# krylea/stylegan3-editing

Measured on AMD Instinct MI355X. Metric: FFHQ-1024 StyleGAN3-T synthesis imgs/sec, higher is better.
Workload: dtype f32

## Files before the change

### include/sg3_ops.h

```cpp
#ifndef SG3_OPS_H
#define SG3_OPS_H

#include <stdint.h>

#ifdef __cplusplus
extern "C" {
#endif

#define SG3_ABI_VERSION 1

#if defined(__GNUC__)
#define SG3_API __attribute__((visibility("default")))
#else
#define SG3_API
#endif

enum {
    SG3_OK          =  0,
    SG3_NO_KERNEL   = -1,
    SG3_BAD_ARG     = -2,
    SG3_HIP_ERROR   = -3,
};

enum {
// ... 18 lines not shown
    int32_t        xH, xW;
    int32_t        yH, yW;
    int64_t        xStride[4];
    int64_t        yStride[4];
    int64_t        bStride;
    int32_t        up, down;
    int32_t        fuW, fuH;
    int32_t        fdW, fdH;
    int32_t        px0, py0;
    int32_t        sH;
    int32_t        sWbytes;
    int32_t        sx, sy;
    int32_t        swLimit;
    float          gain;
    float          slope;
    float          clamp;
    int32_t        flip;
    int32_t        writeSigns;
    int32_t        readSigns;
    float*         ySumPartial;
    int32_t        fdMirror;
    float*         yAbsMaxPartial;
} sg3_filtered_lrelu_params;

SG3_API int sg3_filtered_lrelu(const sg3_filtered_lrelu_params* p, void* stream);

SG3_API int sg3_filtered_lrelu_sum_slots(int N, int C, int yH, int yW, int down);

SG3_API int sg3_filtered_lrelu_finish_partials(const float* sumPartial, const float* absMaxPartial, int N, int C, int slots,
                                               float* db, float* absMax, void* stream);

SG3_API int sg3_filtered_lrelu_planes_per_wave(const sg3_filtered_lrelu_params* p);

SG3_API int sg3_filtered_lrelu_has_kernel(int up, int down, int fuW, int fuH, int fdW, int fdH);

SG3_API int sg3_filtered_lrelu_shape(int xH, int xW, int up, int down,
                             int fuW, int fuH, int fdW, int fdH,
                             int px0, int px1, int py0, int py1,
                             int* yH, int* yW,
                             int* sH, int* sWbytes, int* swLimit);

typedef struct sg3_filtered_lrelu_act_params {
    void*          x;
    uint8_t*       s;
    int32_t        dtype;
    int32_t        N, C, H, W;
    int64_t        xStride[4];
    int32_t        sH, sW;
    int32_t        sx, sy;
    float          gain, slope, clamp;
    int32_t        writeSigns;
    int32_t        readSigns;
} sg3_filtered_lrelu_act_params;

SG3_API int sg3_filtered_lrelu_act(const sg3_filtered_lrelu_act_params* p, void* stream);

typedef struct sg3_upfirdn2d_params {
    const void*    x;
    const float*   f;
    void*          y;
    int32_t        dtype;
    int32_t        N, C, xH, xW, yH, yW;
    int64_t        xStride[4];
    int64_t        yStride[4];
    int32_t        fH, fW;
    int64_t        fStride[2];
// ... 244 lines not shown
```

### stylegan3-editing_amd/csrc/sg3_filtered_lrelu.hip

```cpp
#include "sg3_common.h"
#include <cmath>
#include <cstdlib>

#ifndef SG3_PREFETCH_ROWS
#define SG3_PREFETCH_ROWS 3
#endif
#ifndef SG3_NAN_GUARD
#define SG3_NAN_GUARD 1
#endif

namespace sg3 {

typedef float v2f __attribute__((ext_vector_type(2)));
typedef float v4f __attribute__((ext_vector_type(4)));
typedef __attribute__((address_space(3))) float lds_f;
typedef __attribute__((address_space(3))) v2f lds_v2f;
typedef __attribute__((address_space(3))) v4f lds_v4f;

struct StreamParams {
    const void* x; void* y; const void* b; const float* fu; const float* fd;
    int C, xH, xW, yH, yW;
    int planes;
    long long xsN, xsC, xsH;
    long long ysN, ysC, ysH;
    long long bStride;
    int px0, py0;
    int TW;
    int ox0Base;
    int wideBlocks;
    int CH;
    int nStrips, nChunks;
    int totalBlocks;
    float gain, slope, clamp;
    int flip;
    float* ysum;
    float* ymax;
    unsigned char* s;
    int sH, sWb, sx, sy;
#ifdef SG3_STAMPS
    unsigned long long* stamps;
#endif
};
#ifdef SG3_STAMPS
static unsigned long long* g_stamps = nullptr;
#endif

__device__ __forceinline__ int to_sgpr_i(int v) { return __builtin_amdgcn_readfirstlane(v); }
__device__ __forceinline__ float to_sgpr(float v) {
    return __builtin_bit_cast(float, __builtin_amdgcn_readfirstlane(__builtin_bit_cast(int, v)));
}

__device__ __forceinline__ void wave_lds_sync() {
    __builtin_amdgcn_fence(__ATOMIC_RELEASE, "wavefront");
    __builtin_amdgcn_wave_barrier();
    __builtin_amdgcn_fence(__ATOMIC_ACQUIRE, "wavefront");
}

__device__ __forceinline__ v2f fma2(v2f a, v2f b, v2f c) { return __builtin_elementwise_fma(a, b, c); }
__device__ __forceinline__ v2f splat(float a) { return (v2f){a, a}; }

template <int HALF>
__device__ __forceinline__ v2f fma_tap(v2f a, v2f tapPair, v2f acc) {
    if (HALF == 0) return fma2(a, __builtin_shufflevector(tapPair, tapPair, 0, 0), acc);
    v2f r;
    asm("v_pk_fma_f32 %0, %1, %2, %3 op_sel:[0,1,0] op_sel_hi:[1,1,1]" : "=v"(r) : "v"(a), "s"(tapPair), "v"(acc));
    return r;
}
// ... 96 lines not shown
template <> struct bufio<_Float16> {
    static __device__ __forceinline__ float ld(__amdgpu_buffer_rsrc_t r, int byteOff) {
        return (float)__builtin_bit_cast(_Float16, __builtin_amdgcn_raw_buffer_load_b16(r, byteOff, 0, 0));
    }
    static __device__ __forceinline__ void st1(__amdgpu_buffer_rsrc_t r, int byteOff, float v) {
        __builtin_amdgcn_raw_buffer_store_b16(__builtin_bit_cast(unsigned short, (_Float16)v), r, byteOff, 0, 0);
    }
    static __device__ __forceinline__ void st2(__amdgpu_buffer_rsrc_t r, int byteOff, float a, float b) {
        const unsigned lo = __builtin_bit_cast(unsigned short, (_Float16)a), hi = __builtin_bit_cast(unsigned short, (_Float16)b);
        __builtin_amdgcn_raw_buffer_store_b32(lo | (hi << 16), r, byteOff, 0, 0);
    }
};

template <typename T, int U, int D>
struct WaveState {
    typedef StreamCfg<U, D> Cfg;
    v2f w[6][2];
    v2f xw[6][4];
    v2f acc[6][2];
    float pre[SG3_PREFETCH_ROWS][Cfg::NL];
    float bcol[Cfg::NL];
    int coff[Cfg::NL];
    v2f tuP[Cfg::FU / 2];
    v2f tdP[Cfg::FD / 2];
    unsigned sg[SG3_PREFETCH_ROWS][U];
    float osum;
    float omax;
    int soff;
    int sq;
    int inBase, outBase;
    int ooff[2];
};

template <typename T, int U, int D, int VPH, int RADIAL, int SIGNS, int G = 1>
struct Stream {
    typedef StreamCfg<U, D> Cfg;
    typedef WaveState<T, U, D> State;

    static __device__ __forceinline__ void prefetch(State& st, int slot, const StreamParams& p, const T* __restrict__ plane,
                                                    const unsigned char* __restrict__ splane, int i) {
        const bool rowOk = (unsigned)i < (unsigned)p.xH;
        const T* row = plane + (long long)i * p.xsH;
        const int rowBytes = (G > 1 ? (int)p.xsC + p.xW : p.xW) * (int)sizeof(T);
        const __amdgpu_buffer_rsrc_t rs = __builtin_amdgcn_make_buffer_rsrc((void*)row, (short)0, rowOk ? rowBytes : 0, 0x00020000);
        const float rowFlag = rowOk ? 1.f : 0.f;
#pragma unroll
        for (int q = 0; q < Cfg::NL; q++)
            st.pre[slot][q] = __builtin_fmaf(st.bcol[q], rowFlag, bufio<T>::ld(rs, st.coff[q]));
        if (SIGNS == 2) {
#pragma unroll
            for (int j = 0; j < U; j++) {
                const int sr = U * (i - 5) - (U - 1) + j + p.py0 + p.sy;
                const bool ok = (unsigned)sr < (unsigned)p.sH;
                const unsigned char* srow = splane + (ok ? (long long)sr * p.sWb : 0);
                const __amdgpu_buffer_rsrc_t ss = __builtin_amdgcn_make_buffer_rsrc((void*)srow, (short)0, ok ? p.sWb : 0, 0x00020000);
                const unsigned b0 = __builtin_amdgcn_raw_buffer_load_b8(ss, st.soff, 0, 0);
                const unsigned b1 = __builtin_amdgcn_raw_buffer_load_b8(ss, st.soff + 1, 0, 0);
                st.sg[slot][j] = b0 | (b1 << 8);
            }
        }
    }

    template <int S>
    static __device__ __forceinline__ void step(State& st, const StreamParams& p, const T* __restrict__ plane, T* __restrict__ oplane,
                                                unsigned char* __restrict__ splane, lds_f* sIn, lds_f* sOut, int i, int delta, int lane,
                                                int oy0, int oy1, int ox0, int oxN, bool pairStore, float& liveGain, float& liveGain1, bool wide) {
        constexpr bool RDOWN = RADIAL == 1 || RADIAL == 2 || RADIAL >= 5;
        constexpr bool FOLD = RADIAL >= 5;
        constexpr bool UP2D = RADIAL == 3 || RADIAL == 4;
        wave_lds_sync();
        constexpr int PS = S % SG3_PREFETCH_ROWS;
#pragma unroll
        for (int q = 0; q < Cfg::NL; q++) sIn[lane + 64 * q] = st.pre[PS][q];
        if (SIGNS == 0 && SG3_NAN_GUARD && G > 1) {
#pragma unroll
            for (int q = 0; q < Cfg::NL; q++) {
                unsigned long long m;
                asm("v_cmp_class_f32 %0, %1, %2" : "=s"(m) : "v"(st.pre[PS][q]), "s"(0x207));
                const int n0 = Cfg::PSEG - 64 * q;
                const unsigned long long first = n0 >= 64 ? ~0ull : (n0 <= 0 ? 0ull : ((1ull << (n0 & 63)) - 1ull));
                const unsigned long long mw = q < Cfg::NL - 1 ? m : 0ull;
                liveGain = (wide ? mw : (m & first)) != 0ull ? __builtin_bit_cast(float, 0x7fc00000u) : liveGain;
                liveGain1 = (wide ? mw : (m & ~first)) != 0ull ? __builtin_bit_cast(float, 0x7fc00000u) : liveGain1;
            }
        } else if (SIGNS == 0 && SG3_NAN_GUARD) {
#pragma unroll
            for (int q = 0; q < Cfg::NL - 1; q++) {
                unsigned long long m;
                asm("v_cmp_class_f32 %0, %1, %2" : "=s"(m) : "v"(st.pre[PS][q]), "s"(0x207));
                liveGain = m != 0ull ? __builtin_bit_cast(float, 0x7fc00000u) : liveGain;
            }
        }
        unsigned sgNow[U];
#pragma unroll
        for (int j = 0; j < U; j++) sgNow[j] = SIGNS == 2 ? st.sg[PS][j] : 0u;
        prefetch(st, PS, p, plane, splane, i + SG3_PREFETCH_ROWS);
        wave_lds_sync();
        if (U == 2) {
            float xs[8];
            const volatile lds_v2f* src = reinterpret_cast<const volatile lds_v2f*>(sIn + (G > 1 ? st.inBase : 2 * lane));
#pragma unroll
            for (int q = 0; q < 4; q++) { v2f t = src[q]; xs[2 * q] = t.x; xs[2 * q + 1] = t.y; if (UP2D) st.xw[S][q] = t; }
#pragma unroll
            for (int g = 0; g < 2 && !UP2D; g++) {
                v2f a = splat(xs[g]) * st.tuP[0];
#pragma unroll
                for (int t = 1; t < 6; t++) a = fma2(splat(xs[g + t]), st.tuP[t], a);
                st.w[S][g] = a;
            }
        } else {
            float xs[6];
#pragma unroll
            for (int t = 0; t < 6; t++) xs[t] = sIn[(G > 1 ? st.inBase : lane) + t];
            v2f a0 = splat(xs[0]) * st.tuP[1], a1 = splat(xs[0]) * st.tuP[0];
#pragma unroll
            for (int t = 1; t < 6; t++) {
                a0 = fma2(splat(xs[t]), st.tuP[2 * t + 1], a0);
                a1 = fma2(splat(xs[t]), st.tuP[2 * t], a1);
            }
            st.w[S][0] = a0; st.w[S][1] = a1;
        }
        const float slope = p.slope, clampv = p.clamp / p.gain, gain = p.gain;
        const float gainOut = (SIGNS == 1) ? 1.f : (UP2D ? p.gain * (float)(U * U) : ((SIGNS == 0 && SG3_NAN_GUARD) ? ((G > 1 && lane >= 32) ? liveGain1 : liveGain) : p.gain));
#pragma unroll
        for (int j = 0; j < U; j++) {
            const int kv = U - 1 - j;
            v2f u0, u1;
            TapHalf th[6];
            if (FOLD) {
                const int kp0 = (VPH + S * U + j) % D;
#pragma unroll
                for (int r = 0; r < 6; r++) radial_half_issue(th[r], p.fd, (RADIAL == 6) ? kp0 + r * D : 11 - (kp0 + r * D));
            }
            if (UP2D) {
                constexpr bool FLIPU = RADIAL == 4;
                u0 = splat(0.f); u1 = splat(0.f);
                TapRow rowA, rowB;
                radial_row_issue(rowA, p.fu, FLIPU ? kv : 11 - kv);
#pragma unroll
                for (int t = 0; t < 6; t++) {
                    const int slot = (S + 1 + t) % 6;
                    const int k = kv + 2 * t;
                    TapRow& cur = (t & 1) ? rowB : rowA;
                    TapRow& nxt = (t & 1) ? rowA : rowB;
                    radial_row_wait(cur);
                    if (t < 5) radial_row_issue(nxt, p.fu, FLIPU ? k + 2 : 11 - (k + 2));
#pragma unroll
                    for (int sx = 0; sx < 6; sx++) {
                        const v2f tq = up2d_pair<FLIPU>(cur, sx);
                        u0 = (sx & 1) ? fma_x_tap<1, FLIPU>(st.xw[slot][sx / 2], tq, u0) : fma_x_tap<0, FLIPU>(st.xw[slot][sx / 2], tq, u0);
                        u1 = ((sx + 1) & 1) ? fma_x_tap<1, FLIPU>(st.xw[slot][(sx + 1) / 2], tq, u1) : fma_x_tap<0, FLIPU>(st.xw[slot][(sx + 1) / 2], tq, u1);
                    }
                }
            }
#pragma unroll
            for (int t = 0; t < 6 && !UP2D; t++) {
// ... 8 lines not shown
                } else {
                    u0 = fma_tap<1>(st.w[slot][0], st.tuP[k / 2], u0);
                    u1 = fma_tap<1>(st.w[slot][1], st.tuP[k / 2], u1);
                }
            }
            const int uy = U * (i - 5) - (U - 1) + j + p.py0;
            float a[4] = {u0.x, u0.y, u1.x, u1.y};
            if (SIGNS == 2) {
                const unsigned bits = sgNow[j] >> (2 * st.sq);
#pragma unroll
                for (int c = 0; c < 4; c++) {
                    const unsigned code = bits >> (2 * c);
                    a[c] *= (code & 2u) ? 0.f : ((code & 1u) ? slope : 1.f);
                }
            } else if (SIGNS == 1) {
                unsigned code = 0;
#pragma unroll
                for (int c = 0; c < 4; c++) {
                    const float v = a[c] * gain;
                    const bool neg = v < 0.f;
                    const float lv = neg ? v * slope : v;
                    const bool big = __builtin_fabsf(lv) > p.clamp;
                    a[c] = big ? __builtin_copysignf(p.clamp, lv) : lv;
                    code |= (big ? 2u : (neg ? 1u : 0u)) << (2 * c);
                }
                const int sr = uy + p.sy;
                if (uy >= oy0 * D && uy <= (oy1 - 1) * D + Cfg::FD - 1 && (unsigned)sr < (unsigned)p.sH) {
                    const unsigned nxt = (unsigned)__shfl_down((int)code, 1);
                    const unsigned byte = st.sq == 0 ? code : ((code >> (2 * (4 - st.sq))) | (nxt << (2 * st.sq))) & 0xffu;
                    const int bofs = (st.sq == 0 || lane < 63) ? st.soff + (st.sq ? 1 : 0) : -1;
                    const __amdgpu_buffer_rsrc_t ss = __builtin_amdgcn_make_buffer_rsrc((void*)(splane + (long long)sr * p.sWb), (short)0, p.sWb, 0x00020000);
                    __builtin_amdgcn_raw_buffer_store_b8((unsigned char)byte, ss, bofs, 0, 0);
                }
            } else {
                const v2f s0 = u0 * splat(slope), s1 = u1 * splat(slope);
                a[0] = __builtin_fmaxf(u0.x, s0.x); a[1] = __builtin_fmaxf(u0.y, s0.y); a[2] = __builtin_fmaxf(u1.x, s1.x); a[3] = __builtin_fmaxf(u1.y, s1.y);
#pragma unroll
                for (int c = 0; c < 4; c++) a[c] = __builtin_amdgcn_fmed3f(a[c], -clampv, clampv);
            }
            const v2f r0 = {a[0], a[1]}, r1 = {a[2], a[3]};
            const int kp = (VPH + S * U + j) % D;
            if (RDOWN) {
                lds_f* dstr = sOut + (4 - delta) + (G > 1 ? st.outBase : 4 * lane);
                dstr[0] = r0.x; dstr[1] = r0.y; dstr[2] = r1.x; dstr[3] = r1.y;
                wave_lds_sync();
                const lds_v4f* srcr = reinterpret_cast<const lds_v4f*>(sOut + 4 + (G > 1 ? st.outBase : 4 * lane));
                v2f pr[8];
#pragma unroll
                for (int q = 0; q < 4; q++) { const v4f t = srcr[q]; pr[2 * q] = (v2f){t.x, t.y}; pr[2 * q + 1] = (v2f){t.z, t.w}; }
                wave_lds_sync();
                const int headR = ((VPH + S * U + j) / D) % 6;
                constexpr bool FLIPPED = RADIAL == 2 || RADIAL == 6;
                v2f fo[2][3];
#pragma unroll
                for (int q = 0; q < 3 && FOLD; q++) { fo[0][q] = add_swapped(pr[q], pr[5 - q]); fo[1][q] = add_swapped(pr[q + 1], pr[6 - q]); }
                if (FOLD) radial_half_wait(th);
#pragma unroll
                for (int r = 0; r < 6 && FOLD; r++) {
                    const int slot = (headR + 5 - r) % 6;
                    const int k = kp + r * D;
#pragma unroll
                    for (int q = 0; q < 3; q++) {
                        const v2f tq = q == 0 ? (v2f){th[r].a.x, th[r].a.y} : (q == 1 ? (v2f){th[r].a.z, th[r].a.w} : th[r].b);
                        if (k == 0 && q == 0) {
                            st.acc[slot][0] = radial_mul<true>(fo[0][0], tq);
                            st.acc[slot][1] = radial_mul<true>(fo[1][0], tq);
// ... 94 lines not shown
                        } else {
                            asm volatile("" :: "v"(f0), "v"(f1));
                        }
                        if (false) {
#else
                        if (pairStore) {
#endif
                            bufio<T>::st2(rs, G > 1 ? st.ooff[0] : 2 * lane * (int)sizeof(T), f0, f1);
                        } else {
                            bufio<T>::st1(rs, G > 1 ? st.ooff[0] : 2 * lane * (int)sizeof(T), f0);
                            bufio<T>::st1(rs, G > 1 ? st.ooff[1] : (2 * lane + 1) * (int)sizeof(T), f1);
                        }
                    } else {
                        v2f pr[12];
#pragma unroll
                        for (int q = 0; q < 6; q++) { const v4f t = src[q]; pr[2 * q] = (v2f){t.x, t.y}; pr[2 * q + 1] = (v2f){t.z, t.w}; }
                        v2f y0 = pr[0] * st.tdP[0];
#pragma unroll
                        for (int q = 1; q < Cfg::FD / 2; q++) y0 = fma2(pr[q], st.tdP[q], y0);
                        const float f0 = (y0.x + y0.y) * gainOut;
                        if (SIGNS == 2) {
                            const float m0 = lane < oxN ? f0 : 0.f;
                            st.osum += m0;
                            st.omax = __builtin_fmaxf(st.omax, __builtin_fabsf(m0));
                        }
                        bufio<T>::st1(rs, lane * (int)sizeof(T), f0);
                    }
                    wave_lds_sync();
                }
            }
        }
    }

    static __device__ __forceinline__ void run(const StreamParams& p) {
        static_assert((D == 2 || D == 4) && (6 * U) % D == 0, "streaming kernel: down is 2 or 4");
        constexpr bool RDOWN = RADIAL == 1 || RADIAL == 2 || RADIAL >= 5;
        constexpr bool UP2D = RADIAL == 3 || RADIAL == 4;
        static_assert(RADIAL >= 0 && RADIAL <= 6, "RADIAL: 0 separable, 1/2 12x12 down, 3/4 12x12 up, 5/6 12x12 down with mirror-symmetric rows");
        static_assert(!RDOWN || (D == 2 && SIGNS != 2), "radial down filter: forward passes (plain or sign-writing), down 2");
        static_assert(!UP2D || (U == 2 && SIGNS == 2), "2-D up filter: the adjoint pass, up 2");
        static_assert(G == 1 || (G == 2 && SIGNS == 0 && D == 2), "packed mode: plain forward, down 2, two planes");
#ifdef SG3_FUSION_BOUND
        __shared__ __attribute__((aligned(16))) float lds[Cfg::SIN + Cfg::SOUT + 3 * 128];
#else
        __shared__ __attribute__((aligned(16))) float lds[Cfg::SIN + Cfg::SOUT];
#endif
        lds_f* sIn = (lds_f*)lds;
        lds_f* sOut = (lds_f*)lds + Cfg::SIN;
        const int lane = threadIdx.x;
#ifdef SG3_STAMPS
        const unsigned long long stampC = __builtin_amdgcn_s_memtime(), stampR = __builtin_amdgcn_s_memrealtime();
#endif

        int bid = blockIdx.x;
        {
            const int nb = p.totalBlocks, q = nb >> 3, r = nb & 7, xcd = bid & 7, k = bid >> 3;
            bid = (xcd < r ? xcd * (q + 1) : r * (q + 1) + (xcd - r) * q) + k;
        }
        const bool wide = G > 1 && bid < p.wideBlocks;
        const bool two = G > 1 && !wide;
        const int pbid = two ? bid - p.wideBlocks : bid;
        const int strip = two ? 0 : pbid % p.nStrips;
        const int chunk = two ? pbid % p.nChunks : (pbid / p.nStrips) % p.nChunks;
        const int plane_id = two ? (pbid / p.nChunks) * 2 : pbid / (p.nStrips * p.nChunks);
        const int n = plane_id / p.C, c = plane_id - n * p.C;

// ... 45 lines not shown
            }
            const int ix = ibase + lane + 64 * q;
            st.coff[q] = ix * (int)sizeof(T);
            st.bcol[q] = ((unsigned)ix < (unsigned)p.xW) ? bias : 0.f;
        }
        if (G > 1) {
            const int g = two ? lane >> 5 : 0, ll = two ? lane & 31 : lane;
            st.inBase = g * Cfg::PSEG + Cfg::GROUPS * ll;
            st.outBase = g * Cfg::POSEG + 4 * ll;
            const bool mine = g == 0 || second;
            st.ooff[0] = (mine && 2 * ll < oxN) ? (g * (int)p.ysC + 2 * ll) * (int)sizeof(T) : (int)0x80000000;
            st.ooff[1] = (mine && 2 * ll + 1 < oxN) ? (g * (int)p.ysC + 2 * ll + 1) * (int)sizeof(T) : (int)0x80000000;
        }

        st.osum = 0.f;
        st.omax = 0.f;
        float liveGain = p.gain;
        float liveGain1 = p.gain;
        if (SIGNS) {
            const int c0 = uxs + p.sx;
            st.sq = to_sgpr_i(((c0 % 4) + 4) % 4);
            st.soff = floor_div(c0, 4) + lane;
        } else {
            st.sq = 0; st.soff = 0;
        }

        const int uyA = oy0 * D;
        const int uyB = (oy1 - 1) * D + Cfg::FD - 1;
        int iFirst = ceil_div_s(uyA - p.py0, U);
        if ((U * (iFirst - 5)) % D != 0) iFirst -= 1;
        const int iLast = ceil_div_s(uyB - p.py0, U) + 5;
        const int nBlocks = (iLast - iFirst + 1 + 5) / 6;

#pragma unroll
        for (int s = 0; s < 6; s++) {
            st.w[s][0] = splat(0.f); st.w[s][1] = splat(0.f);
#pragma unroll
            for (int q = 0; q < 4; q++) st.xw[s][q] = splat(0.f);
            st.acc[s][0] = splat(0.f); st.acc[s][1] = splat(0.f);
            if (s < SG3_PREFETCH_ROWS) prefetch(st, s, p, plane, splane, iFirst + s);
        }

        int i = iFirst;
        for (int blk = 0; blk < nBlocks; blk++, i += 6) {
            step<0>(st, p, plane, oplane, splane, sIn, sOut, i + 0, delta, lane, oy0, oy1, ox0, oxN, pairStore, liveGain, liveGain1, wide);
            step<1>(st, p, plane, oplane, splane, sIn, sOut, i + 1, delta, lane, oy0, oy1, ox0, oxN, pairStore, liveGain, liveGain1, wide);
            step<2>(st, p, plane, oplane, splane, sIn, sOut, i + 2, delta, lane, oy0, oy1, ox0, oxN, pairStore, liveGain, liveGain1, wide);
            step<3>(st, p, plane, oplane, splane, sIn, sOut, i + 3, delta, lane, oy0, oy1, ox0, oxN, pairStore, liveGain, liveGain1, wide);
            step<4>(st, p, plane, oplane, splane, sIn, sOut, i + 4, delta, lane, oy0, oy1, ox0, oxN, pairStore, liveGain, liveGain1, wide);
            step<5>(st, p, plane, oplane, splane, sIn, sOut, i + 5, delta, lane, oy0, oy1, ox0, oxN, pairStore, liveGain, liveGain1, wide);
            if ((6 * U / D) % 6 != 0) {
#pragma unroll
                for (int r = 0; r < 3; r++)
#pragma unroll
                    for (int h = 0; h < 2; h++) { const v2f t = st.acc[r][h]; st.acc[r][h] = st.acc[r + 3][h]; st.acc[r + 3][h] = t; }
            }
        }
#ifdef SG3_STAMPS
        if (p.stamps && lane == 0) {
            p.stamps[2 * (long long)blockIdx.x] = __builtin_amdgcn_s_memtime() - stampC;
            p.stamps[2 * (long long)blockIdx.x + 1] = __builtin_amdgcn_s_memrealtime() - stampR;
        }
#endif
        if (SIGNS == 2 && p.ysum) {
            float v = st.osum;
#pragma unroll
            for (int m = 32; m > 0; m >>= 1) v += __shfl_xor(v, m);
            if (lane == 0) p.ysum[(long long)plane_id * (p.nChunks * p.nStrips) + chunk * p.nStrips + strip] = v;
        }
        if (SIGNS == 2 && p.ymax) {
            float v = st.omax;
#pragma unroll
            for (int m = 32; m > 0; m >>= 1) v = __builtin_fmaxf(v, __shfl_xor(v, m));
            if (lane == 0) p.ymax[(long long)plane_id * (p.nChunks * p.nStrips) + chunk * p.nStrips + strip] = v;
        }
    }
};

template <typename T, int U, int D, int VPH, int RADIAL, int SIGNS, int G = 1>
__global__ void __launch_bounds__(64)
flrelu_stream_kernel(StreamParams p) {
    Stream<T, U, D, VPH, RADIAL, SIGNS, G>::run(p);
}

struct PointParams {
    const void* x; void* y; const void* b;
    const float* fu; const float* fd;
    int N, C, H, W;
    long long xs[4], ys[4], bStride;
    int px0, py0, yH, yW;
// ... 39 lines not shown
    if (q.readSigns && q.fdH != 0) return false;
    if (q.readSigns && q.up != 2) return false;
    if (q.down == 4 && !q.readSigns) return false;
    return q.slope >= 0.f && q.slope <= 1.f && q.xStride[3] == 1 && q.yStride[3] == 1 && !(q.clamp < 0.f);
}

static bool pointwise_supported(int up, int down, int fuW, int fuH, int fdW, int fdH) {
    return up == 1 && down == 1 && fuW == 1 && fdW == 1 && fuH <= 1 && fdH <= 1;
}

static void stream_grid(int N, int C, int yH, int yW, int down, int& nStrips, int& TW, int& nChunks, int& CH) {
    const int maxTW = (256 - 6 * down) / down;
    nStrips = ceil_div(yW, maxTW);
    TW = ceil_div(yW, nStrips);
    const long long planes = (long long)N * C;
    const long long wantWaves = 256LL * 16 * 4;
    int n = (int)ceil_div64(wantWaves, planes * nStrips);
    const int maxChunks = max(1, yH / 48);
    if (n > maxChunks) n = maxChunks;
    if (n < 1) n = 1;
    CH = ceil_div(yH, n);
    nChunks = ceil_div(yH, CH);
}

static bool stream_packs_planes(const sg3_filtered_lrelu_params& q, int width) {
    static const bool allowed = [] { const char* e = getenv("SG3_FLRELU_NOPACK"); return !(e && e[0] == '1'); }();
    const long long esz = q.dtype == SG3_F32 ? 4 : 2;
    const long long xsC = q.xStride[1], ysC = q.yStride[1];
    return allowed && !q.readSigns && !q.writeSigns && q.down == 2 && width <= StreamCfg<2, 2>::PACKTW &&
           q.xStride[0] == (long long)q.C * xsC && q.yStride[0] == (long long)q.C * ysC && xsC > 0 && ysC > 0 &&
           (xsC + q.xW) * esz < 0x7fffffffLL && (ysC + q.yW) * esz < 0x7fffffffLL;
}

constexpr int STREAM_FULL_TW = 120;
static int stream_full_strips(int yW, int nStripsEqual) {
    const int nFull = (yW - 1) / STREAM_FULL_TW, rem = yW - nFull * STREAM_FULL_TW;
    return (nFull >= 1 && nFull + 1 == nStripsEqual && rem <= StreamCfg<2, 2>::PACKTW) ? nFull : 0;
}

__global__ void __launch_bounds__(256)
flrelu_finish_partials_kernel(const float* __restrict__ psum, const float* __restrict__ pmax, int N, int C, int slots,
                              float* __restrict__ db, float* __restrict__ amax) {
    __shared__ float red[4];
    float mx = 0.f;
    for (int c = threadIdx.x; c < C; c += 256) {
        float s = 0.f;
        for (int n = 0; n < N; n++) {
            const size_t base = ((size_t)n * C + c) * slots;
            for (int k = 0; k < slots; k++) {
                s += psum[base + k];
                if (pmax) mx = __builtin_fmaxf(mx, pmax[base + k]);
            }
        }
        db[c] = s;
    }
    if (!amax) return;
#pragma unroll
    for (int m = 32; m > 0; m >>= 1) mx = __builtin_fmaxf(mx, __shfl_xor(mx, m));
    if ((threadIdx.x & 63) == 0) red[threadIdx.x >> 6] = mx;
    __syncthreads();
    if (threadIdx.x == 0) amax[0] = __builtin_fmaxf(__builtin_fmaxf(red[0], red[1]), __builtin_fmaxf(red[2], red[3]));
}

template <typename T>
static int launch_stream(const sg3_filtered_lrelu_params& q, hipStream_t st) {
    StreamParams p;
    p.x = q.x; p.y = q.y; p.b = q.b; p.fu = q.fu; p.fd = q.fd;
    p.C = q.C; p.planes = q.N * q.C; p.xH = q.xH; p.xW = q.xW; p.yH = q.yH; p.yW = q.yW;
    p.xsN = q.xStride[0]; p.xsC = q.xStride[1]; p.xsH = q.xStride[2];
    p.ysN = q.yStride[0]; p.ysC = q.yStride[1]; p.ysH = q.yStride[2];
    p.bStride = q.bStride;
    p.px0 = q.px0; p.py0 = q.py0;
    p.gain = q.gain; p.slope = q.slope; p.clamp = q.clamp; p.flip = q.flip;

    p.s = q.s; p.sH = q.sH; p.sWb = q.sWbytes; p.sx = q.sx; p.sy = q.sy;
    p.ysum = q.ySumPartial;
    p.ymax = q.yAbsMaxPartial;
#ifdef SG3_STAMPS
    p.stamps = g_stamps;
#endif
    stream_grid(q.N, q.C, q.yH, q.yW, q.down, p.nStrips, p.TW, p.nChunks, p.CH);
    const long long planes = (long long)q.N * q.C;
    const long long total = planes * p.nStrips * p.nChunks;
    if (total > 0x7fffffffLL) { set_error("filtered_lrelu: grid too large"); return SG3_BAD_ARG; }
    p.totalBlocks = (int)total;

    p.ox0Base = 0;
    const bool packed = p.nStrips == 1 && stream_packs_planes(q, q.yW);
    if (packed) p.totalBlocks = (int)((planes + 1) / 2 * p.nChunks);
    const int remFull = stream_full_strips(q.yW, p.nStrips);
    const bool mixed = !packed && remFull > 0 && stream_packs_planes(q, q.yW - remFull * STREAM_FULL_TW);
    const bool oneLaunch = mixed && (q.fdH == 0 || q.up == 4);
    p.wideBlocks = 0;
    if (mixed) {
        p.nStrips = remFull; p.TW = STREAM_FULL_TW;
        p.totalBlocks = (int)(planes * remFull * p.nChunks);
        if (oneLaunch) {
            p.wideBlocks = p.totalBlocks;
            p.ox0Base = remFull * STREAM_FULL_TW;
            const long long all = (long long)p.totalBlocks + (planes + 1) / 2 * p.nChunks;
            if (all > 0x7fffffffLL) { set_error("filtered_lrelu: grid too large"); return SG3_BAD_ARG; }
            p.totalBlocks = (int)all;
        }
    }

    const int vph = (((q.py0 - (q.up - 1)) % q.down) + q.down) % q.down;
// ... 87 lines not shown
    SG3_REQUIRE(!absMax == !absMaxPartial, "filtered_lrelu_finish_partials: absMaxPartial and absMax come together");
    hipLaunchKernelGGL(flrelu_finish_partials_kernel, dim3(1), dim3(256), 0, (hipStream_t)stream, sumPartial, absMaxPartial, N, C, slots, db, absMax);
    SG3_LAUNCH_CHECK("flrelu_finish_partials_kernel");
    return SG3_OK;
}

int sg3_filtered_lrelu_shape(int xH, int xW, int up, int down, int fuW, int fuH, int fdW, int fdH,
                             int px0, int px1, int py0, int py1, int* yH, int* yW, int* sH, int* sWbytes, int* swLimit) {
    using namespace sg3;
    SG3_REQUIRE(xH > 0 && xW > 0, "x is empty");
    SG3_REQUIRE(up >= 1 && down >= 1, "up and down must be at least 1");
    SG3_REQUIRE(fuW >= 1 && fdW >= 1, "fu and fd must not be empty");
    const int64_t fut_w = fuW - 1, fut_h = (fuH ? fuH : fuW) - 1;
    const int64_t fdt_w = fdW - 1, fdt_h = (fdH ? fdH : fdW) - 1;
    const int64_t cw = (int64_t)xW * up + (px0 + px1) - fut_w;
    const int64_t ch = (int64_t)xH * up + (py0 + py1) - fut_h;
    SG3_REQUIRE(cw > fdt_w && ch > fdt_h, "upsampled buffer must be at least the size of downsampling filter");
    SG3_REQUIRE(cw <= INT32_MAX && ch <= INT32_MAX, "upsampled buffer is too large");
    const int64_t ow = (cw - fdt_w + (down - 1)) / down;
    const int64_t oh = (ch - fdt_h + (down - 1)) / down;
    SG3_REQUIRE(ow > 0 && oh > 0, "output must be at least 1x1");
    const int64_t sw_active = ow * down - (down - 1) + fdt_w;
    const int64_t sh = oh * down - (down - 1) + fdt_h;
    const int64_t sw = (sw_active + 15) & ~(int64_t)15;
    SG3_REQUIRE(sh <= INT32_MAX && (sw >> 2) <= INT32_MAX, "signs is too large");
    if (yH) *yH = (int)oh;
    if (yW) *yW = (int)ow;
    if (sH) *sH = (int)sh;
    if (sWbytes) *sWbytes = (int)(sw >> 2);
    if (swLimit) *swLimit = (int)((sw_active + 3) >> 2);
    return SG3_OK;
}

int sg3_filtered_lrelu_planes_per_wave(const sg3_filtered_lrelu_params* p) {
    using namespace sg3;
    if (!p || (p->dtype != SG3_F32 && p->dtype != SG3_F16)) return 0;
    const bool signs = p->writeSigns || p->readSigns;
    if (!signs && pointwise_supported(p->up, p->down, p->fuW, p->fuH, p->fdW, p->fdH)) return 0;
    if (!(stream_supported(p->up, p->down, p->fuW, p->fuH, p->fdW, p->fdH) && stream_params_ok(*p))) return 0;
    if (p->N <= 0 || p->C <= 0 || p->yH <= 0 || p->yW <= 0) return 0;
    int nStrips, TW, nChunks, CH;
    stream_grid(p->N, p->C, p->yH, p->yW, p->down, nStrips, TW, nChunks, CH);
    if (nStrips == 1) return stream_packs_planes(*p, p->yW) ? 2 : 1;
    const int nFull = stream_full_strips(p->yW, nStrips);
    return (nFull > 0 && stream_packs_planes(*p, p->yW - nFull * STREAM_FULL_TW)) ? 3 : 1;
}

int sg3_filtered_lrelu(const sg3_filtered_lrelu_params* p, void* stream) {
    using namespace sg3;
    SG3_REQUIRE(p && p->x && p->y && p->fu && p->fd, "filtered_lrelu: null tensor");
    SG3_REQUIRE(p->N > 0 && p->C > 0 && p->xH > 0 && p->xW > 0, "filtered_lrelu: x is empty");
    SG3_REQUIRE(p->yH > 0 && p->yW > 0, "filtered_lrelu: output must be at least 1x1");
    SG3_REQUIRE(p->up >= 1 && p->down >= 1, "filtered_lrelu: up and down must be at least 1");
    SG3_REQUIRE(p->dtype == SG3_F32 || p->dtype == SG3_F16, "filtered_lrelu: x must be float16 or float32");
    SG3_REQUIRE(!(p->writeSigns && p->readSigns), "filtered_lrelu: cannot read and write signs in one call");
    hipStream_t st = (hipStream_t)stream;
    const bool signs = p->writeSigns || p->readSigns;
    if (!signs && pointwise_supported(p->up, p->down, p->fuW, p->fuH, p->fdW, p->fdH))
        return p->dtype == SG3_F32 ? launch_pointwise<float>(*p, st) : launch_pointwise<_Float16>(*p, st);
    if (stream_supported(p->up, p->down, p->fuW, p->fuH, p->fdW, p->fdH) && stream_params_ok(*p))
        return p->dtype == SG3_F32 ? launch_stream<float>(*p, st) : launch_stream<_Float16>(*p, st);
    set_error("filtered_lrelu: no fused kernel for up=%d down=%d fu=%dx%d fd=%dx%d signs=%d", p->up, p->down,
              p->fuW, p->fuH, p->fdW, p->fdH, (int)signs);
    return SG3_NO_KERNEL;
}

// ... 2 lines not shown
```

### stylegan3-editing_amd/torch_utils/_sg3abi.py

```python
import ctypes
import os

import torch

_PKG_ROOT = os.path.dirname(os.path.dirname(os.path.abspath(__file__)))
LIB_PATH = os.environ.get('SG3_LIB') or os.path.join(_PKG_ROOT, 'lib', 'libsg3hip.so')

SG3_OK, SG3_NO_KERNEL, SG3_BAD_ARG, SG3_HIP_ERROR = 0, -1, -2, -3
SG3_F32, SG3_F16, SG3_F64 = 0, 1, 2
SG3_CONV_FP32, SG3_CONV_F16X3, SG3_CONV_F16, SG3_CONV_F16X3_F23, SG3_CONV_F16_F23 = 0, 1, 2, 3, 4
_DTYPE = {torch.float32: SG3_F32, torch.float16: SG3_F16, torch.float64: SG3_F64}

c_i32, c_i64, c_f32, c_vp = ctypes.c_int32, ctypes.c_int64, ctypes.c_float, ctypes.c_void_p


class FilteredLreluParams(ctypes.Structure):
    _fields_ = [('x', c_vp), ('y', c_vp), ('b', c_vp), ('s', c_vp), ('fu', c_vp), ('fd', c_vp),
                ('dtype', c_i32), ('N', c_i32), ('C', c_i32), ('xH', c_i32), ('xW', c_i32), ('yH', c_i32), ('yW', c_i32),
                ('xStride', c_i64 * 4), ('yStride', c_i64 * 4), ('bStride', c_i64),
                ('up', c_i32), ('down', c_i32), ('fuW', c_i32), ('fuH', c_i32), ('fdW', c_i32), ('fdH', c_i32),
                ('px0', c_i32), ('py0', c_i32), ('sH', c_i32), ('sWbytes', c_i32), ('sx', c_i32), ('sy', c_i32),
                ('swLimit', c_i32), ('gain', c_f32), ('slope', c_f32), ('clamp', c_f32),
                ('flip', c_i32), ('writeSigns', c_i32), ('readSigns', c_i32), ('ySumPartial', c_vp), ('fdMirror', c_i32), ('yAbsMaxPartial', c_vp)]

# ... 61 lines not shown


class ModconvPrepParams(ctypes.Structure):
    _fields_ = [('w', c_vp), ('s', c_vp), ('wPacked', c_vp), ('wsq', c_vp), ('sIn', c_vp), ('dcoef', c_vp),
                ('inputGain', c_vp), ('inputGainMode', c_i32),
                ('N', c_i32), ('I', c_i32), ('O', c_i32), ('k', c_i32), ('demodulate', c_i32), ('precision', c_i32), ('xBound', c_f32),
                ('xBoundDev', c_vp), ('reuseWeights', c_i32)]


class WgradParams(ctypes.Structure):
    _fields_ = [('x', c_vp), ('dy', c_vp), ('partial', c_vp), ('scaleX', c_vp), ('scaleDy', c_vp), ('dtype', c_i32),
                ('N', c_i32), ('I', c_i32), ('O', c_i32), ('H', c_i32), ('W', c_i32), ('k', c_i32), ('pad', c_i32),
                ('nBands', c_i32), ('nSegGroups', c_i32), ('scalesAreAmax', c_i32)]


class Conv2dParams(ctypes.Structure):
    _fields_ = [('x', c_vp), ('wPacked', c_vp), ('inScale', c_vp), ('inShift', c_vp), ('bias', c_vp), ('slope', c_vp), ('out', c_vp),
                ('N', c_i32), ('I', c_i32), ('O', c_i32), ('H', c_i32), ('W', c_i32), ('k', c_i32), ('stride', c_i32), ('pad', c_i32),
                ('act', c_i32), ('precision', c_i32), ('rangeFlag', c_vp)]


class ImageFinishParams(ctypes.Structure):
    _fields_ = [('x', c_vp), ('xStride', c_i64 * 4), ('y', c_vp), ('yStride', c_i64 * 4),
                ('B', c_i32), ('H', c_i32), ('W', c_i32), ('h', c_i32), ('w', c_i32),
                ('boundsH', c_vp), ('coeffsH', c_vp), ('kH', c_i32), ('boundsV', c_vp), ('coeffsV', c_vp), ('kV', c_i32)]


EXPORTS = [
    ('sg3_abi_version', ctypes.c_int, []),
    ('sg3_last_error', ctypes.c_char_p, []),
    ('sg3_device_count', ctypes.c_int, []),
    ('sg3_filtered_lrelu', ctypes.c_int, [ctypes.POINTER(FilteredLreluParams), c_vp]),
    ('sg3_filtered_lrelu_planes_per_wave', ctypes.c_int, [ctypes.POINTER(FilteredLreluParams)]),
    ('sg3_filtered_lrelu_has_kernel', ctypes.c_int, [ctypes.c_int] * 6),
    ('sg3_filtered_lrelu_sum_slots', ctypes.c_int, [ctypes.c_int] * 5),
    ('sg3_filtered_lrelu_finish_partials', ctypes.c_int, [c_vp, c_vp, ctypes.c_int, ctypes.c_int, ctypes.c_int, c_vp, c_vp, c_vp]),
    ('sg3_filtered_lrelu_shape', ctypes.c_int, [ctypes.c_int] * 12 + [ctypes.POINTER(ctypes.c_int)] * 5),
    ('sg3_filtered_lrelu_act', ctypes.c_int, [ctypes.POINTER(FilteredLreluActParams), c_vp]),
    ('sg3_upfirdn2d', ctypes.c_int, [ctypes.POINTER(Upfirdn2dParams), c_vp]),
    ('sg3_upfirdn2d_shape', ctypes.c_int, [ctypes.c_int] * 12 + [ctypes.POINTER(ctypes.c_int)] * 2),
    ('sg3_bias_act', ctypes.c_int, [ctypes.POINTER(BiasActParams), c_vp]),
    ('sg3_modconv_packed_floats', ctypes.c_int64, [ctypes.c_int] * 4),
    ('sg3_modulated_conv2d', ctypes.c_int, [ctypes.POINTER(ModconvParams), c_vp]),
    ('sg3_modconv_split_scratch_floats', ctypes.c_int64, [ctypes.POINTER(ModconvParams)]),
    ('sg3_modconv_f23_supported', ctypes.c_int, [ctypes.c_int] * 8),
    ('sg3_modconv_f23_force_rows', ctypes.c_int, [ctypes.c_int]),
    ('sg3_fourier_features', ctypes.c_int, [ctypes.POINTER(FourierParams), c_vp]),
    ('sg3_input_transform', ctypes.c_int, [ctypes.POINTER(InputTransformParams), c_vp]),
    ('sg3_affine_batch', ctypes.c_int, [ctypes.POINTER(AffineBatchParams), c_vp]),
    ('sg3_se_residual', ctypes.c_int, [ctypes.POINTER(SeParams), c_vp]),
    ('sg3_unfold3x3s2', ctypes.c_int, [ctypes.POINTER(UnfoldParams), c_vp]),
    ('sg3_head_gemm_packed_halfs', ctypes.c_int64, [ctypes.c_int] * 3),
    ('sg3_head_gemm_pack', ctypes.c_int, [c_vp, c_vp, ctypes.c_int, ctypes.c_int, ctypes.c_int, c_vp, c_vp]),
    ('sg3_head_gemm', ctypes.c_int, [ctypes.POINTER(HeadGemmParams), c_vp]),
    ('sg3_modulation_backward', ctypes.c_int, [ctypes.POINTER(ModgradParams), c_vp]),
    ('sg3_modconv_transpose_weights', ctypes.c_int, [c_vp, c_vp, ctypes.c_int, ctypes.c_int, ctypes.c_int, ctypes.c_int, c_vp]),
    ('sg3_modulated_conv2d_prep', ctypes.c_int, [ctypes.POINTER(ModconvPrepParams), c_vp]),
    ('sg3_modulated_conv2d_prep_batch', ctypes.c_int, [ctypes.POINTER(ModconvPrepParams), ctypes.c_int, c_vp]),
    ('sg3_conv2d', ctypes.c_int, [ctypes.POINTER(Conv2dParams), c_vp]),
    ('sg3_conv2d_wgrad_splits', ctypes.c_int, [ctypes.c_int] * 7 + [ctypes.POINTER(ctypes.c_int)] * 2),
    ('sg3_conv2d_wgrad', ctypes.c_int, [ctypes.POINTER(WgradParams), c_vp]),
    ('sg3_conv2d_pack', ctypes.c_int, [c_vp, c_vp, c_vp, ctypes.c_int, ctypes.c_int, ctypes.c_int, ctypes.c_int, c_vp]),
    ('sg3_resample_coeffs', ctypes.c_int, [ctypes.c_int32, ctypes.c_int32, c_vp, c_vp]),
    ('sg3_image_finish', ctypes.c_int, [ctypes.POINTER(ImageFinishParams), c_vp]),
]

# ... 58 lines not shown
```

Baseline: 445.0.

## Add bounded-input fast path for filtered lrelu using single med3 clamp

```diff
diff --git a/include/sg3_ops.h b/include/sg3_ops.h
--- a/include/sg3_ops.h
+++ b/include/sg3_ops.h
@@ -74,6 +74,8 @@
 
 SG3_API int sg3_filtered_lrelu_planes_per_wave(const sg3_filtered_lrelu_params* p);
 
+SG3_API float sg3_filtered_lrelu_fast_threshold(const float* fu, int fuW, int up, float gain, float slope, float clamp);
+
 SG3_API int sg3_filtered_lrelu_has_kernel(int up, int down, int fuW, int fuH, int fdW, int fdH);
 
 SG3_API int sg3_filtered_lrelu_shape(int xH, int xW, int up, int down,
diff --git a/stylegan3-editing_amd/csrc/sg3_filtered_lrelu.hip b/stylegan3-editing_amd/csrc/sg3_filtered_lrelu.hip
--- a/stylegan3-editing_amd/csrc/sg3_filtered_lrelu.hip
+++ b/stylegan3-editing_amd/csrc/sg3_filtered_lrelu.hip
@@ -33,6 +33,7 @@
     int totalBlocks;
     float gain, slope, clamp;
     int flip;
+    int fastAct;
     float* ysum;
     float* ymax;
     unsigned char* s;
@@ -195,6 +196,20 @@
     int ooff[2];
 };
 
+__host__ __device__ static inline float fast_threshold(const float* fu, int taps, int up, float gain, float slope, float clamp) {
+    const float clampv = clamp / gain;
+    if (!(clampv > 0.f)) return -1.f;
+    float hs = 0.f;
+    for (int ph = 0; ph < up; ph++) {
+        float s = 0.f;
+        for (int k = ph; k < taps; k += up) s += fabsf(fu[k]);
+        hs = fmaxf(hs, s);
+    }
+    hs *= (float)up;
+    const float hv = hs * hs;
+    return fminf(clampv / (slope * hv), 0x1p124f / fmaxf(hv, 1.f)) * 0.9999f;
+}
+
 template <typename T, int U, int D, int VPH, int RADIAL, int SIGNS, int G = 1>
 struct Stream {
     typedef StreamCfg<U, D> Cfg;
@@ -224,10 +239,11 @@
         }
     }
 
-    template <int S>
+    template <int S, bool FAST>
     static __device__ __forceinline__ void step(State& st, const StreamParams& p, const T* __restrict__ plane, T* __restrict__ oplane,
                                                 unsigned char* __restrict__ splane, lds_f* sIn, lds_f* sOut, int i, int delta, int lane,
-                                                int oy0, int oy1, int ox0, int oxN, bool pairStore, float& liveGain, float& liveGain1, bool wide) {
+                                                int oy0, int oy1, int ox0, int oxN, bool pairStore, float& liveGain, float& liveGain1, bool wide,
+                                                float fastT) {
         constexpr bool RDOWN = RADIAL == 1 || RADIAL == 2 || RADIAL >= 5;
         constexpr bool FOLD = RADIAL >= 5;
         constexpr bool UP2D = RADIAL == 3 || RADIAL == 4;
@@ -235,7 +251,15 @@
         constexpr int PS = S % SG3_PREFETCH_ROWS;
 #pragma unroll
         for (int q = 0; q < Cfg::NL; q++) sIn[lane + 64 * q] = st.pre[PS][q];
-        if (SIGNS == 0 && SG3_NAN_GUARD && G > 1) {
+        if (SIGNS == 0 && FAST) {
+#pragma unroll
+            for (int q = 0; q < Cfg::NL; q++) {
+                unsigned long long m;
+                if (RADIAL) asm("v_cmp_nle_f32_e64 %0, |%1|, %2" : "=s"(m) : "v"(st.pre[PS][q]), "v"(fastT));
+                else        asm("v_cmp_nle_f32_e64 %0, |%1|, %2" : "=s"(m) : "v"(st.pre[PS][q]), "s"(fastT));
+                liveGain = m != 0ull ? 0.f : liveGain;
+            }
+        } else if (SIGNS == 0 && SG3_NAN_GUARD && G > 1) {
 #pragma unroll
             for (int q = 0; q < Cfg::NL; q++) {
                 unsigned long long m;
@@ -284,7 +308,8 @@
             st.w[S][0] = a0; st.w[S][1] = a1;
         }
         const float slope = p.slope, clampv = p.clamp / p.gain, gain = p.gain;
-        const float gainOut = (SIGNS == 1) ? 1.f : (UP2D ? p.gain * (float)(U * U) : ((SIGNS == 0 && SG3_NAN_GUARD) ? ((G > 1 && lane >= 32) ? liveGain1 : liveGain) : p.gain));
+        const float gainOut = (SIGNS == 1) ? 1.f : (UP2D ? p.gain * (float)(U * U) :
+                              ((SIGNS == 0 && (SG3_NAN_GUARD || FAST)) ? ((G > 1 && lane >= 32 && !FAST) ? liveGain1 : liveGain) : p.gain));
 #pragma unroll
         for (int j = 0; j < U; j++) {
             const int kv = U - 1 - j;
@@ -359,6 +384,10 @@
                     const __amdgpu_buffer_rsrc_t ss = __builtin_amdgcn_make_buffer_rsrc((void*)(splane + (long long)sr * p.sWb), (short)0, p.sWb, 0x00020000);
                     __builtin_amdgcn_raw_buffer_store_b8((unsigned char)byte, ss, bofs, 0, 0);
                 }
+            } else if (FAST) {
+                const v2f s0 = u0 * splat(slope), s1 = u1 * splat(slope);
+                a[0] = __builtin_amdgcn_fmed3f(u0.x, s0.x, clampv); a[1] = __builtin_amdgcn_fmed3f(u0.y, s0.y, clampv);
+                a[2] = __builtin_amdgcn_fmed3f(u1.x, s1.x, clampv); a[3] = __builtin_amdgcn_fmed3f(u1.y, s1.y, clampv);
             } else {
                 const v2f s0 = u0 * splat(slope), s1 = u1 * splat(slope);
                 a[0] = __builtin_fmaxf(u0.x, s0.x); a[1] = __builtin_fmaxf(u0.y, s0.y); a[2] = __builtin_fmaxf(u1.x, s1.x); a[3] = __builtin_fmaxf(u1.y, s1.y);
@@ -519,6 +548,37 @@
         }
     }
 
+    template <bool FAST>
+    static __device__ __forceinline__ void stream_chunk(State& st, const StreamParams& p, const T* __restrict__ plane, T* __restrict__ oplane,
+                                                        unsigned char* __restrict__ splane, lds_f* sIn, lds_f* sOut, int iFirst, int nBlocks,
+                                                        int delta, int lane, int oy0, int oy1, int ox0, int oxN, bool pairStore, float& liveGain,
+                                                        float& liveGain1, bool wide, float fastT) {
+#pragma unroll
+        for (int s = 0; s < 6; s++) {
+            st.w[s][0] = splat(0.f); st.w[s][1] = splat(0.f);
+#pragma unroll
+            for (int q = 0; q < 4; q++) st.xw[s][q] = splat(0.f);
+            st.acc[s][0] = splat(0.f); st.acc[s][1] = splat(0.f);
+            if (s < SG3_PREFETCH_ROWS) prefetch(st, s, p, plane, splane, iFirst + s);
+        }
+
+        int i = iFirst;
+        for (int blk = 0; blk < nBlocks; blk++, i += 6) {
+            step<0, FAST>(st, p, plane, oplane, splane, sIn, sOut, i + 0, delta, lane, oy0, oy1, ox0, oxN, pairStore, liveGain, liveGain1, wide, fastT);
+            step<1, FAST>(st, p, plane, oplane, splane, sIn, sOut, i + 1, delta, lane, oy0, oy1, ox0, oxN, pairStore, liveGain, liveGain1, wide, fastT);
+            step<2, FAST>(st, p, plane, oplane, splane, sIn, sOut, i + 2, delta, lane, oy0, oy1, ox0, oxN, pairStore, liveGain, liveGain1, wide, fastT);
+            step<3, FAST>(st, p, plane, oplane, splane, sIn, sOut, i + 3, delta, lane, oy0, oy1, ox0, oxN, pairStore, liveGain, liveGain1, wide, fastT);
+            step<4, FAST>(st, p, plane, oplane, splane, sIn, sOut, i + 4, delta, lane, oy0, oy1, ox0, oxN, pairStore, liveGain, liveGain1, wide, fastT);
+            step<5, FAST>(st, p, plane, oplane, splane, sIn, sOut, i + 5, delta, lane, oy0, oy1, ox0, oxN, pairStore, liveGain, liveGain1, wide, fastT);
+            if ((6 * U / D) % 6 != 0) {
+#pragma unroll
+                for (int r = 0; r < 3; r++)
+#pragma unroll
+                    for (int h = 0; h < 2; h++) { const v2f t = st.acc[r][h]; st.acc[r][h] = st.acc[r + 3][h]; st.acc[r + 3][h] = t; }
+            }
+        }
+    }
+
     static __device__ __forceinline__ void run(const StreamParams& p) {
         static_assert((D == 2 || D == 4) && (6 * U) % D == 0, "streaming kernel: down is 2 or 4");
         constexpr bool RDOWN = RADIAL == 1 || RADIAL == 2 || RADIAL >= 5;
@@ -630,30 +690,19 @@
         const int iLast = ceil_div_s(uyB - p.py0, U) + 5;
         const int nBlocks = (iLast - iFirst + 1 + 5) / 6;
 
-#pragma unroll
-        for (int s = 0; s < 6; s++) {
-            st.w[s][0] = splat(0.f); st.w[s][1] = splat(0.f);
-#pragma unroll
-            for (int q = 0; q < 4; q++) st.xw[s][q] = splat(0.f);
-            st.acc[s][0] = splat(0.f); st.acc[s][1] = splat(0.f);
-            if (s < SG3_PREFETCH_ROWS) prefetch(st, s, p, plane, splane, iFirst + s);
-        }
-
-        int i = iFirst;
-        for (int blk = 0; blk < nBlocks; blk++, i += 6) {
-            step<0>(st, p, plane, oplane, splane, sIn, sOut, i + 0, delta, lane, oy0, oy1, ox0, oxN, pairStore, liveGain, liveGain1, wide);
-            step<1>(st, p, plane, oplane, splane, sIn, sOut, i + 1, delta, lane, oy0, oy1, ox0, oxN, pairStore, liveGain, liveGain1, wide);
-            step<2>(st, p, plane, oplane, splane, sIn, sOut, i + 2, delta, lane, oy0, oy1, ox0, oxN, pairStore, liveGain, liveGain1, wide);
-            step<3>(st, p, plane, oplane, splane, sIn, sOut, i + 3, delta, lane, oy0, oy1, ox0, oxN, pairStore, liveGain, liveGain1, wide);
-            step<4>(st, p, plane, oplane, splane, sIn, sOut, i + 4, delta, lane, oy0, oy1, ox0, oxN, pairStore, liveGain, liveGain1, wide);
-            step<5>(st, p, plane, oplane, splane, sIn, sOut, i + 5, delta, lane, oy0, oy1, ox0, oxN, pairStore, liveGain, liveGain1, wide);
-            if ((6 * U / D) % 6 != 0) {
-#pragma unroll
-                for (int r = 0; r < 3; r++)
-#pragma unroll
-                    for (int h = 0; h < 2; h++) { const v2f t = st.acc[r][h]; st.acc[r][h] = st.acc[r + 3][h]; st.acc[r + 3][h] = t; }
-            }
-        }
+        bool slow = true;
+        if constexpr (SIGNS == 0) {
+            const float fastT = p.fastAct ? to_sgpr(fast_threshold(p.fu, Cfg::FU, U, p.gain, p.slope, p.clamp)) : -1.f;
+            if (fastT > 0.f) {
+                float fastGain = p.gain, unused = p.gain;
+                stream_chunk<true>(st, p, plane, oplane, splane, sIn, sOut, iFirst, nBlocks, delta, lane, oy0, oy1, ox0, oxN, pairStore, fastGain,
+                                   unused, wide, fastT);
+                slow = fastGain != p.gain;
+            }
+        }
+        if (slow)
+            stream_chunk<false>(st, p, plane, oplane, splane, sIn, sOut, iFirst, nBlocks, delta, lane, oy0, oy1, ox0, oxN, pairStore, liveGain, liveGain1,
+                                wide, -1.f);
 #ifdef SG3_STAMPS
         if (p.stamps && lane == 0) {
             p.stamps[2 * (long long)blockIdx.x] = __builtin_amdgcn_s_memtime() - stampC;
@@ -759,6 +808,11 @@
            (xsC + q.xW) * esz < 0x7fffffffLL && (ysC + q.yW) * esz < 0x7fffffffLL;
 }
 
+static bool stream_fast_activation(const sg3_filtered_lrelu_params& q) {
+    const char* e = getenv("SG3_FLRELU_SLOWACT");
+    return !(e && e[0] == '1') && !q.readSigns && !q.writeSigns && q.gain > 0.f && q.gain < INFINITY && q.clamp >= 0.f;
+}
+
 constexpr int STREAM_FULL_TW = 120;
 static int stream_full_strips(int yW, int nStripsEqual) {
     const int nFull = (yW - 1) / STREAM_FULL_TW, rem = yW - nFull * STREAM_FULL_TW;
@@ -799,6 +853,7 @@
     p.bStride = q.bStride;
     p.px0 = q.px0; p.py0 = q.py0;
     p.gain = q.gain; p.slope = q.slope; p.clamp = q.clamp; p.flip = q.flip;
+    p.fastAct = stream_fast_activation(q) ? 1 : 0;
 
     p.s = q.s; p.sH = q.sH; p.sWb = q.sWbytes; p.sx = q.sx; p.sy = q.sy;
     p.ysum = q.ySumPartial;
@@ -952,6 +1007,11 @@
     return SG3_OK;
 }
 
+float sg3_filtered_lrelu_fast_threshold(const float* fu, int fuW, int up, float gain, float slope, float clamp) {
+    if (!fu || up < 1 || fuW < up) return -1.f;
+    return sg3::fast_threshold(fu, fuW, up, gain, slope, clamp);
+}
+
 int sg3_filtered_lrelu_planes_per_wave(const sg3_filtered_lrelu_params* p) {
     using namespace sg3;
     if (!p || (p->dtype != SG3_F32 && p->dtype != SG3_F16)) return 0;
diff --git a/stylegan3-editing_amd/torch_utils/_sg3abi.py b/stylegan3-editing_amd/torch_utils/_sg3abi.py
--- a/stylegan3-editing_amd/torch_utils/_sg3abi.py
+++ b/stylegan3-editing_amd/torch_utils/_sg3abi.py
@@ -117,6 +117,7 @@
     ('sg3_device_count', ctypes.c_int, []),
     ('sg3_filtered_lrelu', ctypes.c_int, [ctypes.POINTER(FilteredLreluParams), c_vp]),
     ('sg3_filtered_lrelu_planes_per_wave', ctypes.c_int, [ctypes.POINTER(FilteredLreluParams)]),
+    ('sg3_filtered_lrelu_fast_threshold', ctypes.c_float, [c_vp, ctypes.c_int, ctypes.c_int, ctypes.c_float, ctypes.c_float, ctypes.c_float]),
     ('sg3_filtered_lrelu_has_kernel', ctypes.c_int, [ctypes.c_int] * 6),
     ('sg3_filtered_lrelu_sum_slots', ctypes.c_int, [ctypes.c_int] * 5),
     ('sg3_filtered_lrelu_finish_partials', ctypes.c_int, [c_vp, c_vp, ctypes.c_int, ctypes.c_int, ctypes.c_int, c_vp, c_vp, c_vp]),
```

Result: faster. 452.3, median of 6 (+1.6%).
